# graphdeco-inria/reduced-3dgs

Hardware: AMD Instinct MI355X
Metric: train iters/s (fwd+bwd) + Mpix/s render, 500k Gaussians @1600x1062 (higher is better)
Workload: dtype f32

## Files before the change

reduced-3dgs_amd/csrc/common.h:

```cpp
#pragma once
#include <hip/hip_runtime.h>
#include <stddef.h>
#include <stdint.h>

#include <functional>
#include <stdexcept>
#include <string>

#include "gauss_math.h"
#include "param_math.h"

namespace r3 {

constexpr size_t kAlign = 256;
constexpr int kPairGrad = 9;
#ifndef R3_ACC_STRIDE
#define R3_ACC_STRIDE 12
#endif
#ifndef R3_PAIR_STRIDE
#define R3_PAIR_STRIDE 12
#endif
#ifdef R3_WP_VEC
constexpr int kPieceStride = 12;
#else
constexpr int kPieceStride = 9;
#endif
constexpr int kAccStride = R3_ACC_STRIDE;
constexpr int kPairStride = R3_PAIR_STRIDE;

constexpr int kPreBlockSize = 256;
struct PrePartial {
    uint32_t visible;
    uint32_t num_rendered;
    uint32_t depth_max;
    uint32_t depth_inv_min;
    uint32_t binned;
    uint32_t rendered_ref;
    uint32_t pad[2];
};
static_assert(sizeof(PrePartial) == 32, "two 16-byte loads per partial");
struct GeomHeader {
    uint32_t visible, num_rendered, depth_max, depth_inv_min;
    uint32_t num_pairs;
    uint32_t reserve;
    uint32_t sort_overflow;
    uint32_t binned;
    uint32_t rendered_ref;
    uint32_t sh_cache;
    uint32_t ckpt;
    uint32_t ckpt_thr;
    uint32_t pad[52];
};
static_assert(sizeof(GeomHeader) == 256, "header = 256 B");
inline size_t pre_partials(size_t P) { return (P + kPreBlockSize - 1) / kPreBlockSize; }

struct PassInfo {
    uint32_t seq;
    uint32_t num_rendered;
    uint32_t visible;
    uint32_t reserve;
    uint32_t sort_overflow;
    uint32_t sort_seq;
    uint32_t pairs;
    uint32_t pad;
};
static_assert(sizeof(PassInfo) == 32, "PassInfo = 32 B");

constexpr int kMinDepthBuckets = 1024;
constexpr int kMaxDepthBuckets = 16384;
constexpr int kBucketCap = 4096;
#ifndef R3_HIST_BATCH
#define R3_HIST_BATCH 4096
#endif
constexpr int kHistBatch = R3_HIST_BATCH;
inline size_t depth_hist_per_block(size_t P)
{
    const size_t want = (P + 255) / 256;
    const size_t per = ((want + kHistBatch - 1) / kHistBatch) * kHistBatch;
    return per < (size_t)kHistBatch ? (size_t)kHistBatch : per;
}
int depth_bucket_load();
inline int depth_bucket_count(size_t P)
{
    int nb = kMinDepthBuckets;
    const size_t load = (size_t)depth_bucket_load() * (P > (1u << 22) ? 8 : P > (1u << 20) ? 4 : 1);
    while (nb < kMaxDepthBuckets && P / (size_t)nb > load) nb <<= 1;
    return nb;
}
struct DepthSortScratch {
    uint32_t depth_max, depth_inv_min;
    uint32_t big_count, pad_;
    unsigned long long total[kMaxDepthBuckets + 1];
    uint32_t start[kMaxDepthBuckets + 2];
    uint32_t tile_base[kMaxDepthBuckets + 2];
    uint32_t big_list[kMaxDepthBuckets];
};
inline size_t depth_hist_rows(size_t P) { const size_t per = depth_hist_per_block(P); return (P + per - 1) / per; }

struct Carver {
    char* p;
    explicit Carver(char* base)
        : p(reinterpret_cast<char*>((reinterpret_cast<uintptr_t>(base) + kAlign - 1) & ~(uintptr_t)(kAlign - 1)))
    {
    }
    template <class T>
    T* take(size_t count)
    {
        T* r = reinterpret_cast<T*>(p);
        size_t bytes = (count * sizeof(T) + kAlign - 1) & ~(kAlign - 1);
        p += bytes;
        return r;
    }
};

struct GeomState {
    GeomHeader* header;
    PrePartial* partials;
    DepthSortScratch* dsort;
    unsigned long long* hist_rows;
    uint32_t* hist_base;
    GRec* rec;
    float* acc;
    ushort4* rect;
    uint32_t* depth_key;
    uint32_t* tiles;
    uint32_t* key_sorted;
    uint32_t* bucket_id;
    uint4* rec16;
    ushort4* rect_sorted;
    uint4* rec16_b;
    uint32_t* order;
    uint32_t* offsets;
    int* radii_internal;
    float* sh_ddir;
    uint32_t* ovf_key;
    uint32_t* ovf_id;
    char* temp;
    size_t temp_bytes;
    static GeomState carve(char* base, size_t P, size_t temp_bytes)
    {
        Carver c(base);
        GeomState g;
        const size_t nb = (size_t)depth_bucket_count(P);
        g.header = c.take<GeomHeader>(1);
        g.partials = c.take<PrePartial>(pre_partials(P));
        g.dsort = c.take<DepthSortScratch>(1);
        g.hist_rows = c.take<unsigned long long>(depth_hist_rows(P) * (nb + 1));
        g.hist_base = c.take<uint32_t>(depth_hist_rows(P) * (nb + 1));
        g.rec = c.take<GRec>(P);
        g.acc = c.take<float>(P * kAccStride);
        g.rect = c.take<ushort4>(P);
        g.depth_key = c.take<uint32_t>(P);
        g.tiles = c.take<uint32_t>(P);
        g.key_sorted = c.take<uint32_t>(P);
        g.bucket_id = c.take<uint32_t>(P);
        g.order = c.take<uint32_t>(P);
        g.offsets = c.take<uint32_t>(P);
        g.radii_internal = c.take<int>(P);
        g.ovf_key = c.take<uint32_t>(P);
        g.ovf_id = c.take<uint32_t>(P);
        g.rec16 = c.take<uint4>(P);
        g.rect_sorted = c.take<ushort4>(P);
        g.rec16_b = c.take<uint4>(P);
        g.temp = c.take<char>(temp_bytes);
        g.temp_bytes = temp_bytes;
        g.lean_end = c.p;
        g.sh_ddir = c.take<float>(P * 9);
        g.end = c.p;
        return g;
    }
    char* lean_end;
    char* end;
};

inline uint32_t higher_msb(uint32_t n)
{
    uint32_t msb = sizeof(n) * 4, step = msb;
    while (step > 1) {
        step /= 2;
        if (n >> msb)
            msb += step;
        else
            msb -= step;
    }
    if (n >> msb) msb++;
    return msb;
}

constexpr int kRadixBlock = 2048;
constexpr int kMaxRadixBins = 256;
constexpr int kMaxRadixPasses = 3;
struct PairLayout {
    int tile_bits;
    int rank_bits;
    int wide;
    int passes;
    int digit_bits;
};
PairLayout pair_layout(int P, size_t n_tiles);

inline uint32_t radix_row_stride(size_t R)
{
    return (uint32_t)(((R + kRadixBlock - 1) / kRadixBlock + 3) & ~(size_t)3);
}

constexpr int kBwdSegMinLog2 = 7;
constexpr int kBwdSegMaxLog2 = 8;
constexpr int kBwdSegMax = 32;
constexpr int kFwdCkptMax = 256;
constexpr uint32_t kUnitTileBits = 20;
R3_HD size_t ckpt_slot(uint32_t first, uint32_t k, uint32_t tile, uint32_t seg_log2) { return (size_t)(first >> seg_log2) + tile + k; }
inline size_t ckpt_slots(size_t R, size_t Tn) { return (R >> kBwdSegMinLog2) + Tn + 2; }
constexpr uint32_t kOrderLists = 8, kListBlock = 4, kListBlockTiles = kListBlock * kListBlock;
struct TileGrid {
    uint32_t gx, gy;
    R3_HD size_t n() const { return (size_t)gx * gy; }
    R3_HD uint32_t blocks_x() const { return (gx + kListBlock - 1) / kListBlock; }
    R3_HD uint32_t blocks() const { return blocks_x() * ((gy + kListBlock - 1) / kListBlock); }
    R3_HD uint32_t list_slots(uint32_t list) const
    {
        return blocks() > list ? (blocks() - list + kOrderLists - 1) / kOrderLists * kListBlockTiles : 0u;
    }
    R3_HD uint32_t list_tile(uint32_t list, uint32_t j) const
    {
        const uint32_t k = j / kListBlockTiles * kOrderLists + list, o = j % kListBlockTiles, bx = blocks_x();
        const uint32_t tx = k % bx * kListBlock + o % kListBlock, ty = k / bx * kListBlock + o / kListBlock;
        return tx < gx && ty < gy ? ty * gx + tx : 0xFFFFFFFFu;
    }
    R3_HD uint32_t list_tiles_max() const
    {
        const size_t m = (size_t)((blocks() + kOrderLists - 1) / kOrderLists) * kListBlockTiles;
        return (uint32_t)(m < n() ? m : n());
    }
};
R3_HD uint32_t bwd_list_fit(uint32_t pairs, const TileGrid& g)
{
    const size_t extra = (size_t)pairs >> kBwdSegMinLog2, most = 8 * g.n();
    return g.list_tiles_max() + (uint32_t)((extra < most ? extra : most) / kOrderLists);
}
inline uint32_t bwd_units_cap(uint32_t reserve, const TileGrid& g) { return (bwd_list_fit(reserve, g) + 1u) * kOrderLists; }
int bwd_segment_log2();
int bwd_segment_factor_pct();

struct BinState {
    uint32_t* point_list;
    float* pair_grad;
    float* wave_part;
    unsigned char* pair_flag;
    uint32_t* pair_rank;
    char* words_a;
    char* words_b;
    char* words_c;
    uint32_t* radix_rows;
    uint32_t* radix_base;
    uint32_t* radix_total;
    uint32_t* block_first;
    unsigned long long* quad_masks;
    uint32_t* unit_order;
    float4* ckpt;
    char* end;
    static BinState carve(char* base, size_t R, int wide, const TileGrid& grid)
    {
        const size_t Tn = grid.n();
        Carver c(base);
        BinState b;
        b.point_list = c.take<uint32_t>(R);
        b.pair_grad = c.take<float>(R * kPairStride);
        b.wave_part = c.take<float>((R / 64 + 1) * 2 * kPieceStride);
        b.pair_flag = c.take<unsigned char>(R);
        if (wide == 1) {
            b.pair_rank = c.take<uint32_t>(R);
            b.words_a = reinterpret_cast<char*>(c.take<unsigned long long>(R));
            b.words_b = reinterpret_cast<char*>(c.take<unsigned long long>(R));
            b.words_c = nullptr;
        } else if (wide == 2) {
            b.words_a = reinterpret_cast<char*>(c.take<unsigned long long>(R));
            b.words_b = reinterpret_cast<char*>(c.take<unsigned long long>(R));
            b.words_c = nullptr;
            b.pair_rank = reinterpret_cast<uint32_t*>(b.words_a);
        } else {
            b.words_a = reinterpret_cast<char*>(c.take<uint32_t>(R));
            b.words_b = reinterpret_cast<char*>(c.take<uint32_t>(R));
            b.words_c = reinterpret_cast<char*>(c.take<uint32_t>(R));
            b.pair_rank = reinterpret_cast<uint32_t*>(b.words_a);
        }
        b.radix_rows = c.take<uint32_t>((size_t)kMaxRadixBins * radix_row_stride(R));
        b.radix_base = c.take<uint32_t>((size_t)kMaxRadixBins * radix_row_stride(R));
        b.radix_total = c.take<uint32_t>(kMaxRadixPasses * kMaxRadixBins);
        b.quad_masks = c.take<unsigned long long>((R / 64 + Tn + 2) * 4);
        b.block_first = c.take<uint32_t>(R / kRadixBlock + 2);
        b.unit_order = c.take<uint32_t>((size_t)bwd_units_cap((uint32_t)R, grid) + 2 * kOrderLists);
        b.ckpt = c.take<float4>(ckpt_slots(R, Tn) * 256);
        b.end = c.p;
        return b;
    }
};

R3_HD size_t quad_mask_slot(uint32_t first, uint32_t chunk, uint32_t tile)
{
    return (size_t)(first >> 6) + chunk + tile;
}

struct ImageState {
    float* final_T;
    uint32_t* n_contrib;
    uint2* ranges;
    uint32_t* quad_depth;
    uint32_t* tile_order;
    char* end;
    static ImageState carve(char* base, size_t N, size_t Tn)
    {
        Carver c(base);
        ImageState s;
        s.final_T = c.take<float>(N);
        s.n_contrib = c.take<uint32_t>(N);
        s.ranges = c.take<uint2>(Tn);
        s.quad_depth = c.take<uint32_t>(Tn * 4);
        s.tile_order = c.take<uint32_t>(Tn);
        s.end = c.p;
        return s;
    }
};

template <class S, class... A>
size_t required_bytes(A... a)
{
    S s = S::carve(nullptr, a...);
    return (size_t)reinterpret_cast<uintptr_t>(s.end) + kAlign;
}

size_t depth_sort_temp_bytes(size_t P);

inline uint32_t grid_pairs_for(uint32_t reserve)
{
    const uint64_t g = (uint64_t)reserve * 7 / 10;
    return (uint32_t)(g < 1024 ? (reserve < 1024 ? reserve : 1024) : g);
}

struct Error : std::runtime_error {
    using std::runtime_error::runtime_error;
};

#if defined(__HIP_DEVICE_COMPILE__)
#define R3_GLOBAL __attribute__((address_space(1)))
#else
#define R3_GLOBAL
#endif
template <class T>
__device__ __forceinline__ R3_GLOBAL T* global_ptr(T* p)
{
    return (R3_GLOBAL T*)p;
}

int guarded_call(const std::function<int()>& f);

#define R3_HIP(expr)                                                                                   \
    do {                                                                                               \
        hipError_t e_ = (expr);                                                                        \
        if (e_ != hipSuccess)                                                                          \
            throw r3::Error(std::string(#expr) + " failed: " + hipGetErrorString(e_) + " (" + __FILE__ + \
                            ":" + std::to_string(__LINE__) + ")");                                     \
    } while (0)

inline void check_launch(const char* what, hipStream_t s, bool debug)
{
    hipError_t e = hipGetLastError();
    if (e != hipSuccess) throw Error(std::string(what) + ": launch failed: " + hipGetErrorString(e));
    if (debug) {
        e = hipStreamSynchronize(s);
        if (e != hipSuccess) throw Error(std::string(what) + ": " + hipGetErrorString(e));
    }
}

struct ViewParams {
    const float* view;
    const float* proj;
    const float* campos;
    const float* bg;
    float tan_fovx, tan_fovy;
    int W, H;
    float scale_modifier;
};

__device__ __forceinline__ Camera load_camera(const ViewParams& v)
{
    Camera c;
#pragma unroll
    for (int k = 0; k < 16; k++) {
        c.view[k] = v.view[k];
        c.proj[k] = v.proj[k];
    }
    c.campos[0] = v.campos[0];
    c.campos[1] = v.campos[1];
    c.campos[2] = v.campos[2];
    c.tan_fovx = v.tan_fovx;
    c.tan_fovy = v.tan_fovy;
    c.focal_y = v.H / (2.0f * v.tan_fovy);
    c.focal_x = v.W / (2.0f * v.tan_fovx);
    c.W = v.W;
    c.H = v.H;
    c.gx = (v.W + kTile - 1) / kTile;
    c.gy = (v.H + kTile - 1) / kTile;
    c.scale_modifier = v.scale_modifier;
    return c;
}

struct FwdInputs {
    int P, M;
    const int* degrees;
    const float* means3D;
    const float* scales;
    const float* rotations;
    const float* opacities;
    const float* shs;
    const float* cov3D_precomp;
    const float* colors_precomp;
    const int* coeffs_num;
    const int* per_band_count;
    const int* cumsum_count;
};

struct BwdOutputs {
    float* dL_dmean2D;
    float* dL_dopacity;
    float* dL_dcolor;
    float* dL_dmean3D;
    float* dL_dcov3D;
    float* dL_dsh;
    float* dL_dscale;
    float* dL_drot;
    float* dL_dconic;
};

struct PreArgs {
    FwdInputs in;
    ViewParams view;
    GRec* rec;
    ushort4* rect;
    uint32_t* depth_key;
    uint32_t* tiles;
    PrePartial* partials;
    int* radii;
    int color_blocks;
    int tight;
    float* sh_ddir;
};
struct HeaderArgs {
    const PrePartial* parts;
    int n_parts;
    GeomHeader* hdr;
    PassInfo* info;
    uint32_t ticket;
    uint32_t reserve;
    uint32_t stamp_sort;
    uint32_t sh_cache;
    uint32_t ckpt;
    uint32_t ckpt_factor_pct, n_tiles;
};
struct DepthArgs {
    int P, nb, rows, per_block;
    int fuse_header;
    const uint32_t* key;
    const uint32_t* tiles;
    GeomHeader* hdr;
    PassInfo* info;
    uint32_t ticket;
    DepthSortScratch* ds;
    unsigned long long* hist_rows;
    uint32_t* hist_base;
    uint32_t* key_sorted;
    uint32_t* bucket_id;
    uint32_t* ovf_key;
    uint32_t* ovf_id;
    const ushort4* rect;
    uint4* rec16;
    uint4* rec16_b;
    ushort4* rect_sorted;
    uint32_t* order;
    uint32_t* offsets;
    uint32_t* block_first;
    uint32_t block_cap;
};
struct EmitArgs {
    int P, gx;
    const GeomHeader* hdr;
    const uint32_t* order;
    const uint32_t* offsets;
    const uint32_t* block_first;
    const ushort4* rect;
    const ushort4* rect_sorted;
    GRec* rec;
    int rank_bits, digit_bits;
    char* words_out;
    uint32_t cap;
    uint32_t* pair_rank;
    uint2* ranges;
    uint32_t n_tiles;
    uint32_t* radix_rows;
    uint32_t row_stride;
};
struct RadixArgs {
    const GeomHeader* hdr;
    const char* in;
    char* out;
    uint32_t* ids_out;
    uint32_t cap;
    int shift, digit_bits;
    int rank_bits, tile_shift;
    uint32_t* rows;
    uint32_t* base;
    uint32_t* total;
    uint32_t row_stride;
};
struct RangesArgs {
    const GeomHeader* hdr;
    const char* sorted;
    uint32_t cap;
    int rank_bits;
    const uint32_t* order;
    uint32_t* point_list;
    uint2* ranges;
    unsigned char* pair_flag;
};
struct BlendFwdArgs {
    const uint2* ranges;
    const uint32_t* point_list;
    const GRec* rec;
    int W, H, gx;
    uint32_t nblocks;
    const float* bg;
    float* out_color;
    float* final_T;
    uint32_t* n_contrib;
    int* touched;
    float* transmittance;
    unsigned long long* quad_masks;
    uint32_t* quad_depth;
    float4* ckpt;
    const GeomHeader* hdr;
};
struct BlendBwdArgs {
    const uint2* ranges;
    const uint32_t* point_list;
    const GRec* rec;
    const float* final_T;
    const uint32_t* n_contrib;
    const float* dL_dpix;
    int W, H, gx;
    uint32_t nblocks;
    const float* bg;
    float* pair_grad;
    unsigned char* pair_flag;
    const unsigned long long* quad_masks;
    uint32_t* tile_order;
    uint32_t units_cap;
    const uint32_t* quad_depth;
    const float4* ckpt;
    const GeomHeader* hdr;
    int segments;
};
struct PairReduceArgs {
    const GeomHeader* hdr;
    const float* pair_grad;
    unsigned char* pair_flag;
    const uint32_t* pair_rank;
    uint32_t rank_mask;
    const uint32_t* order;
    const GRec* rec;
    const uint32_t* tiles;
    float* acc;
    float* wave_part;
    uint32_t stamp0, stamp1;
};
struct PreBwdArgs {
    FwdInputs in;
    ViewParams view;
    const int* radii;
    const GRec* rec;
    const uint32_t* tiles;
    const float* acc;
    const float* wave_part;
    const float* pair_grad;
    uint32_t stamp0, stamp1;
    const GeomHeader* header;
    float lambda_sh;
    const float* sh_ddir;
    int stagger;
    BwdOutputs out;
    const float* shs_rest;
    float* dL_dsh_rest;
};

struct FwdPassArgs {
    PreArgs pre;
    HeaderArgs header;
    DepthArgs depth;
    EmitArgs emit;
    RadixArgs radix[kMaxRadixPasses];
    RangesArgs ranges;
    BlendFwdArgs blend;
    const float* shs_rest;
};
struct BwdPassArgs {
    BlendBwdArgs blend;
    PairReduceArgs reduce;
    PreBwdArgs pre;
};
static_assert(sizeof(FwdPassArgs) <= 3072 && sizeof(BwdPassArgs) <= 3072, "pass blocks travel as by-value kernel arguments");

struct FwdPlan {
    int P, M, W, H, gx, gy;
    uint32_t reserve;
    uint32_t grid_pairs;
    PairLayout layout;
    int nb;
    int ragged, counters;
    int color_in_geom;
    int color_side;
    int fwd_ppl;
    int color_grid;
    int color_fuse;
    int color_split[3];
    int generic_depth_sort;
    int tight;
    int raw_params;
};
struct BwdPlan {
    int P, M, W, H, gx, gy;
    uint32_t reserve, grid_pairs;
    uint32_t units_cap;
    PairLayout layout;
    int bwd_ppl;
    int has_pairs;
    int f64_chain;
    int raw_params;
};

enum Stage { kPre = 0, kDepthSort, kBinning, kBlendFwd, kBlendBwd, kPreBwd, kColor, kBlendBwdKernel, kNumStages };

void issue_preprocess_geom(const FwdPlan& p, FwdPassArgs* dst, const FwdPassArgs& v, hipStream_t s);
void issue_preprocess_color(const FwdPlan& p, const PreArgs* a, hipStream_t s);
void launch_mark_visible(int P, const float* means3D, const float* view, bool* present, hipStream_t s);
void launch_activate_params(int P, const float* scaling_raw, const float* rotation_raw, float* scales, float* rotations,
                            hipStream_t s);

void issue_header_reduce(const HeaderArgs* a, hipStream_t s);
void prepare_depth_bucket_sort(int nb);
void issue_depth_sort_and_color(const FwdPlan& p, const FwdPassArgs* a, hipStream_t s);
void run_generic_depth_sort(int P, GeomState& g, hipStream_t s);
void issue_tile_binning(const FwdPlan& p, const FwdPassArgs* a, hipStream_t s);
const char* sorted_words(const BinState& b, const PairLayout& l);
void launch_export_keys(int P, int R, int cap, size_t n_tiles, const BinState& b, const GeomState& g, uint64_t* keys_out,
                        hipStream_t s);
void launch_export_point_list(int count, const uint32_t* point_list, const GeomHeader* hdr, uint32_t* out, hipStream_t s);

void issue_blend_forward(const FwdPlan& p, const BlendFwdArgs* a, hipStream_t s);
void issue_unit_order(const BwdPlan& p, BwdPassArgs* dst, const BwdPassArgs& v, hipStream_t s);
void issue_blend_backward(const BwdPlan& p, BwdPassArgs* dst, const BwdPassArgs& v, hipStream_t s);
void issue_pair_reduce(const BwdPlan& p, const PairReduceArgs* a, hipStream_t s);
void issue_preprocess_backward(const BwdPlan& p, const PreBwdArgs* a, hipStream_t s);

void launch_colour_variance_accumulate(int P, const int* D, int M, int max_sh_deg, const float* means3D,
                                       const float* cam_pos, const float* shs, const int* radii, const int* touched,
                                       const float* transmittance, float* wSum, float* wSumSq, float* mean,
                                       float* variance, float* accum, hipStream_t s);

int env_int(const char* env, int dflt, int lo, int hi);

#if defined(__HIPCC__)
template <class Block>
__device__ __forceinline__ void install_block_from_kernarg(Block* dst, int tid, int nthreads)
{
    static_assert(alignof(Block) == 8 && sizeof(Block) % 4 == 0, "kernarg layout: [dst (8 B)][block]");
#if defined(__HIP_DEVICE_COMPILE__)
    typedef const uint32_t __attribute__((address_space(4))) * KernargWords;
    KernargWords src = (KernargWords)__builtin_amdgcn_kernarg_segment_ptr() + sizeof(Block*) / 4;
    uint32_t* d = reinterpret_cast<uint32_t*>(dst);
    for (uint32_t k = (uint32_t)tid; k < sizeof(Block) / 4; k += (uint32_t)nthreads) d[k] = src[k];
#endif
}
#endif

}
```

reduced-3dgs_amd/csrc/preprocess_bwd.hip:

```cpp
#include "common.h"

namespace r3 {

#ifndef R3_PREBWD_BLOCK
#define R3_PREBWD_BLOCK 64
#endif
constexpr int kBwdBlock = R3_PREBWD_BLOCK;
constexpr int kBwdWaveShFloats = 64 * 48 + (64 * 48) / 32;

template <bool ROWS48>
__device__ __forceinline__ int bskew(int e)
{
    if (ROWS48) return e + (int)(((uint32_t)e * 43691u) >> 21);
    return e + (e >> 5);
}

template <bool ROWS48>
struct ShRowLdsRW {
    float* base;
    int roff;
    __device__ __forceinline__ float at(int e) const { return ROWS48 ? base[e] : base[bskew<false>(roff + e)]; }
    __device__ __forceinline__ void put(int e, float v) const
    {
        if (ROWS48)
            base[e] = v;
        else
            base[bskew<false>(roff + e)] = v;
    }
};

template <bool ROWS48>
__device__ __forceinline__ int split_lds_index(int f, int rl, int k0, int M)
{
    if (ROWS48) {
        const int row = k0 == 0 ? (int)(((uint32_t)f * 43691u) >> 17) : (int)(((uint32_t)f * 46604u) >> 21);
        return f + (49 - rl) * row + k0;
    }
    const int row = f / rl;
    return bskew<false>(row * 3 * M + k0 + (f - row * rl));
}

template <bool ROWS48, bool VEC>
__device__ __forceinline__ void stage_split_span(const float* __restrict__ src, int len, int rl, int k0, int M, float* lds,
                                                 int lane)
{
    if (VEC) {
        constexpr int kBatch = 6;
        const float4* src4 = reinterpret_cast<const float4*>(src);
        const int n4 = len >> 2;
        for (int base = 0; base < n4; base += 64 * kBatch) {
            float4 v[kBatch];
#pragma unroll
            for (int k = 0; k < kBatch; k++) {
                const int e4 = base + k * 64 + lane;
                v[k] = e4 < n4 ? src4[e4] : make_float4(0.f, 0.f, 0.f, 0.f);
            }
#pragma unroll
            for (int k = 0; k < kBatch; k++) {
                const int e4 = base + k * 64 + lane;
                if (e4 < n4) {
                    const int f = e4 << 2;
                    lds[split_lds_index<ROWS48>(f, rl, k0, M)] = v[k].x;
                    lds[split_lds_index<ROWS48>(f + 1, rl, k0, M)] = v[k].y;
                    lds[split_lds_index<ROWS48>(f + 2, rl, k0, M)] = v[k].z;
                    lds[split_lds_index<ROWS48>(f + 3, rl, k0, M)] = v[k].w;
                }
            }
        }
    } else {
        for (int f = lane; f < len; f += 64) lds[split_lds_index<ROWS48>(f, rl, k0, M)] = src[f];
    }
}

template <bool ROWS48, bool VEC>
__device__ __forceinline__ void unstage_split_span(float* __restrict__ dst, int len, int rl, int k0, int M, const float* lds,
                                                   int lane, bool rows)
{
    if (VEC) {
        float4* dst4 = reinterpret_cast<float4*>(dst);
        const int n4 = len >> 2;
        if (rows) {
            for (int e4 = lane; e4 < n4; e4 += 64) {
                const int f = e4 << 2;
                dst4[e4] = make_float4(lds[split_lds_index<ROWS48>(f, rl, k0, M)], lds[split_lds_index<ROWS48>(f + 1, rl, k0, M)],
                                       lds[split_lds_index<ROWS48>(f + 2, rl, k0, M)], lds[split_lds_index<ROWS48>(f + 3, rl, k0, M)]);
            }
        } else {
            for (int e4 = lane; e4 < n4; e4 += 64) dst4[e4] = make_float4(0.f, 0.f, 0.f, 0.f);
        }
    } else if (rows) {
        for (int f = lane; f < len; f += 64) dst[f] = lds[split_lds_index<ROWS48>(f, rl, k0, M)];
    } else {
        for (int f = lane; f < len; f += 64) dst[f] = 0.f;
    }
}

constexpr int kReduceGroups = 1;

__device__ __forceinline__ void pair_reduce_group(const PairReduceArgs& a, uint32_t e, int lane, bool valid, uint32_t key,
                                                  float (&v)[kPairGrad], uint32_t key_before, uint32_t key_after)
{
#define R3_SEG_STEP(CTRL, RMASK)                                                                                          \
    {                                                                                                                     \
        const uint32_t ku = (uint32_t)__builtin_amdgcn_update_dpp((int)~key, (int)key, CTRL, RMASK, 0xf, false);          \
        const bool take = ku == key;                                                                                      \
        _Pragma("unroll") for (int k = 0; k < kPairGrad; k++)                                                             \
        {                                                                                                                 \
            const float vu = __builtin_bit_cast(                                                                          \
                float, __builtin_amdgcn_update_dpp(0, __builtin_bit_cast(int, v[k]), CTRL, RMASK, 0xf, false));           \
            if (take) v[k] += vu;                                                                                         \
        }                                                                                                                 \
    }
    R3_SEG_STEP(0x111, 0xf)
    R3_SEG_STEP(0x112, 0xf)
    R3_SEG_STEP(0x114, 0xf)
    R3_SEG_STEP(0x118, 0xf)
    R3_SEG_STEP(0x142, 0xa)
    R3_SEG_STEP(0x143, 0xc)
#undef R3_SEG_STEP
    const uint32_t knext = (uint32_t)__shfl_down((int)key, 1);
    const uint32_t key0 = (uint32_t)__builtin_amdgcn_readfirstlane((int)key);
    if (valid && (lane == 63 || knext != key)) {
        const uint32_t gid = a.order ? a.order[key] : key;
        const bool from_before = key == key0 && key_before == key;
        const bool into_next = lane == 63 && key_after == key;
#ifdef R3_EXP_PR_NOSTORE
        if (v[0] != 12345.678f) return;
#endif
        if (!from_before && !into_next) {
#ifdef R3_ACC_IN_SLAB
            float4* dst = reinterpret_cast<float4*>(const_cast<float*>(a.pair_grad) + (size_t)e * kPairStride);
#else
            float4* dst = reinterpret_cast<float4*>(a.acc + (size_t)gid * kAccStride);
#endif
#ifndef R3_NO_ZERO_ROW_SKIP
            bool nz = false;
#pragma unroll
            for (int k = 0; k < kPairGrad; k++) nz |= v[k] != 0.f;
            if (nz) {
                dst[0] = make_float4(v[0], v[1], v[2], v[3]);
                dst[1] = make_float4(v[4], v[5], v[6], v[7]);
                dst[2] = make_float4(v[8], __uint_as_float(a.stamp0), __uint_as_float(a.stamp1), 0.f);
            }
#else
            dst[0] = make_float4(v[0], v[1], v[2], v[3]);
            dst[1] = make_float4(v[4], v[5], v[6], v[7]);
            dst[2] = make_float4(v[8], 0.f, 0.f, 0.f);
            if (kAccStride >= 16) dst[3] = make_float4(0.f, 0.f, 0.f, 0.f);
#endif
        } else {
            float* wp = a.wave_part + (size_t)(e >> 6) * 2 * kPieceStride;
#ifdef R3_WP_VEC
            if (from_before) {
                float4* w4 = reinterpret_cast<float4*>(wp);
                w4[0] = make_float4(v[0], v[1], v[2], v[3]);
                w4[1] = make_float4(v[4], v[5], v[6], v[7]);
                w4[2] = make_float4(v[8], 0.f, 0.f, 0.f);
            }
            if (into_next) {
                float4* w4 = reinterpret_cast<float4*>(wp + kPieceStride);
                w4[0] = make_float4(v[0], v[1], v[2], v[3]);
                w4[1] = make_float4(v[4], v[5], v[6], v[7]);
                w4[2] = make_float4(v[8], 0.f, 0.f, 0.f);
            }
#else
            if (from_before) {
#pragma unroll
                for (int k = 0; k < kPairGrad; k++) wp[k] = v[k];
            }
            if (into_next) {
#pragma unroll
                for (int k = 0; k < kPairGrad; k++) wp[kPieceStride + k] = v[k];
            }
#endif
        }
    }
}

#ifdef R3_PR_WAVES
__attribute__((amdgpu_waves_per_eu(R3_PR_WAVES, R3_PR_WAVES)))
#endif
__global__ __launch_bounds__(256) void pair_reduce_kernel(const PairReduceArgs* __restrict__ ap)
{
    const PairReduceArgs a = *ap;
    const uint32_t R = a.hdr->num_pairs;
    constexpr uint32_t kPerBlock = 256u * kReduceGroups;
  for (uint32_t blk = blockIdx.x; blk * kPerBlock < R; blk += gridDim.x) {
    const float* __restrict__ pair_grad = a.pair_grad;
    unsigned char* __restrict__ pair_flag = a.pair_flag;
    const uint32_t* __restrict__ pair_gid = a.pair_rank;
    const uint32_t rank_mask = a.rank_mask;
    const int lane = threadIdx.x & 63, wave = threadIdx.x >> 6;
    const uint32_t e0 = blk * kPerBlock + (uint32_t)wave * (64u * kReduceGroups) + (uint32_t)lane;
    float v[kReduceGroups][kPairGrad];
    uint32_t key[kReduceGroups], kb[kReduceGroups], ka[kReduceGroups];
    bool flag[kReduceGroups];
#pragma unroll
    for (int g = 0; g < kReduceGroups; g++) {
        const uint32_t e = e0 + 64u * g, gbase = e & ~63u;
        key[g] = e < R ? pair_gid[e] & rank_mask : 0xFFFFFFFFu;
        flag[g] = e < R && pair_flag[e] != 0;
        kb[g] = gbase > 0u && gbase < R ? pair_gid[gbase - 1u] & rank_mask : 0xFFFFFFFFu;
        ka[g] = gbase + 64u < R ? pair_gid[gbase + 64u] & rank_mask : 0xFFFFFFFFu;
    }
#pragma unroll
    for (int g = 0; g < kReduceGroups; g++) {
        const uint32_t e = e0 + 64u * g;
#pragma unroll
        for (int k = 0; k < kPairGrad; k++) v[g][k] = 0.f;
#ifdef R3_EXP_PR_NOLOAD
        if (flag[g] && e == 0xFFFFFFF0u) {
#else
        if (flag[g]) {
#endif
            pair_flag[e] = 0;
            const float4* src = reinterpret_cast<const float4*>(pair_grad + (size_t)e * kPairStride);
            const float4 r0 = src[0], r1 = src[1];
            v[g][0] = r0.x; v[g][1] = r0.y; v[g][2] = r0.z; v[g][3] = r0.w;
            v[g][4] = r1.x; v[g][5] = r1.y; v[g][6] = r1.z; v[g][7] = r1.w;
            v[g][8] = src[2].x;
        }
    }
#pragma unroll
    for (int g = 0; g < kReduceGroups; g++) {
        const uint32_t e = e0 + 64u * g;
        pair_reduce_group(a, e, lane, e < R, key[g], v[g], kb[g], ka[g]);
    }
  }
}

void issue_pair_reduce(const BwdPlan& p, const PairReduceArgs* a, hipStream_t s)
{
    if (!p.has_pairs) return;
    constexpr uint32_t per = 256u * kReduceGroups;
    hipLaunchKernelGGL(pair_reduce_kernel, dim3((p.grid_pairs + per - 1u) / per), dim3(256), 0, s, a);
}

template <bool ROWS48, bool F64, bool RAW = false>
__global__ __launch_bounds__(kBwdBlock) void preprocess_bwd_kernel(const PreBwdArgs* __restrict__ ap)
{
    __shared__ float s_sh[kBwdBlock / 64][kBwdWaveShFloats];
    const PreBwdArgs a = *ap;
    const int tid = threadIdx.x, lane = tid & 63, wave = tid >> 6;
    const int P = a.in.P, M = a.in.M;
    const int i = blockIdx.x * kBwdBlock + tid;
    const bool valid = i < P;
    const int wave_first = blockIdx.x * kBwdBlock + wave * 64;
    const Camera cam = load_camera(a.view);
    const bool has_sh = a.in.shs != nullptr;

    const bool vis = valid && a.radii[i] > 0;
    const int nrows = max(0, min(64, P - wave_first));
    const int span_len = has_sh ? nrows * 3 * M : 0;
    const long span_first = 3L * M * wave_first;
    float* lds = s_sh[wave];
    const bool wave_vis = __ballot(vis) != 0ull;
    const bool cached = has_sh && a.sh_ddir != nullptr && a.header->sh_cache != 0u;
    if (!cached && a.stagger > 0 && blockIdx.x < 768u * (256 / kBwdBlock)) {
        const int steps = (int)(blockIdx.x / (256u * (256 / kBwdBlock))) * a.stagger;
        for (int k = 0; k < steps; k += 127) __builtin_amdgcn_s_sleep(127);
    }
    if (RAW) {
        if (wave_vis && !cached) {
            const int rl = 3 * (M - 1);
            if ((nrows & 3) == 0) {
                stage_split_span<ROWS48, true>(a.in.shs + 3L * wave_first, 3 * nrows, 3, 0, M, lds, lane);
                if (M > 1) stage_split_span<ROWS48, true>(a.shs_rest + (long)rl * wave_first, rl * nrows, rl, 3, M, lds, lane);
            } else {
                stage_split_span<ROWS48, false>(a.in.shs + 3L * wave_first, 3 * nrows, 3, 0, M, lds, lane);
                if (M > 1) stage_split_span<ROWS48, false>(a.shs_rest + (long)rl * wave_first, rl * nrows, rl, 3, M, lds, lane);
            }
        }
    } else if (has_sh && wave_vis && !cached) {
        const float* src = a.in.shs + span_first;
        if (((span_first | span_len) & 3) == 0) {
            const float4* src4 = reinterpret_cast<const float4*>(src);
            const int n4 = span_len >> 2;
            constexpr int kBatch = 6;
            for (int base = 0; base < n4; base += 64 * kBatch) {
                float4 v[kBatch];
#pragma unroll
                for (int k = 0; k < kBatch; k++) {
                    const int e4 = base + k * 64 + lane;
                    v[k] = e4 < n4 ? src4[e4] : make_float4(0.f, 0.f, 0.f, 0.f);
                }
#pragma unroll
                for (int k = 0; k < kBatch; k++) {
                    const int e4 = base + k * 64 + lane;
                    if (e4 < n4) {
                        const int e = e4 << 2;
                        if (ROWS48) {
                            float* d = lds + bskew<true>(e);
                            d[0] = v[k].x;
                            d[1] = v[k].y;
                            d[2] = v[k].z;
                            d[3] = v[k].w;
                        } else {
                            lds[bskew<false>(e)] = v[k].x;
                            lds[bskew<false>(e + 1)] = v[k].y;
                            lds[bskew<false>(e + 2)] = v[k].z;
                            lds[bskew<false>(e + 3)] = v[k].w;
                        }
                    }
                }
            }
        } else {
            for (int e = lane; e < span_len; e += 64) lds[bskew<ROWS48>(e)] = src[e];
        }
    }
    __syncthreads();

    float dmean[3] = {0.f, 0.f, 0.f}, dcov6[6] = {0.f, 0.f, 0.f, 0.f, 0.f, 0.f};
    float dscale[3] = {0.f, 0.f, 0.f}, dq[4] = {0.f, 0.f, 0.f, 0.f};
    float g2x = 0.f, g2y = 0.f, dop = 0.f, dcol[3] = {0.f, 0.f, 0.f}, gcon[3] = {0.f, 0.f, 0.f};
    int K = 0;
    const ShRowLdsRW<ROWS48> row{ROWS48 ? lds + 49 * lane : lds, ROWS48 ? 0 : lane * 3 * M};
    if (vis) {
        const float mx = a.in.means3D[3 * i], my = a.in.means3D[3 * i + 1], mz = a.in.means3D[3 * i + 2];
        const GRec r = a.rec[i];
        const uint32_t start = r.pair_start, ntile = a.tiles[i];
        if (a.wave_part && start != 0xFFFFFFFFu && start + ntile <= a.header->num_pairs) {
            float acc9[kPairGrad];
            const uint32_t last = start + ntile - 1u;
            const uint32_t w0 = start >> 6, w1 = last >> 6;
            if (w0 == w1) {
#ifdef R3_ACC_IN_SLAB
                const float4* ap = reinterpret_cast<const float4*>(a.pair_grad + (size_t)last * kPairStride);
#else
                const float4* ap = reinterpret_cast<const float4*>(a.acc + (size_t)i * kAccStride);
#endif
                float4 a0 = ap[0], a1 = ap[1], a2 = ap[2];
#ifndef R3_NO_ZERO_ROW_SKIP
                if (__float_as_uint(a2.y) != a.stamp0 || __float_as_uint(a2.z) != a.stamp1)
                    a0 = a1 = a2 = make_float4(0.f, 0.f, 0.f, 0.f);
#endif
                acc9[0] = a0.x; acc9[1] = a0.y; acc9[2] = a0.z; acc9[3] = a0.w;
                acc9[4] = a1.x; acc9[5] = a1.y; acc9[6] = a1.z; acc9[7] = a1.w;
                acc9[8] = a2.x;
            } else {
#ifdef R3_WP_VEC
                const float4* w4 = reinterpret_cast<const float4*>(a.wave_part + (size_t)w0 * 2 * kPieceStride + kPieceStride);
                float4 p0 = w4[0], p1 = w4[1], p2 = w4[2];
                acc9[0] = p0.x; acc9[1] = p0.y; acc9[2] = p0.z; acc9[3] = p0.w;
                acc9[4] = p1.x; acc9[5] = p1.y; acc9[6] = p1.z; acc9[7] = p1.w;
                acc9[8] = p2.x;
                for (uint32_t w = w0 + 1; w <= w1; w++) {
                    w4 = reinterpret_cast<const float4*>(a.wave_part + (size_t)w * 2 * kPieceStride);
                    p0 = w4[0]; p1 = w4[1]; p2 = w4[2];
                    acc9[0] += p0.x; acc9[1] += p0.y; acc9[2] += p0.z; acc9[3] += p0.w;
                    acc9[4] += p1.x; acc9[5] += p1.y; acc9[6] += p1.z; acc9[7] += p1.w;
                    acc9[8] += p2.x;
                }
#else
                const float* wp = a.wave_part + (size_t)w0 * 2 * kPieceStride + kPieceStride;
#pragma unroll
                for (int k = 0; k < kPairGrad; k++) acc9[k] = wp[k];
                for (uint32_t w = w0 + 1; w <= w1; w++) {
                    wp = a.wave_part + (size_t)w * 2 * kPieceStride;
#pragma unroll
                    for (int k = 0; k < kPairGrad; k++) acc9[k] += wp[k];
                }
#endif
            }
            g2x = acc9[0];
            g2y = acc9[1];
            gcon[0] = acc9[2];
            gcon[1] = acc9[3];
            gcon[2] = acc9[4];
            dop = acc9[5];
            dcol[0] = acc9[6];
            dcol[1] = acc9[7];
            dcol[2] = acc9[8];
        }
        float sc[3] = {0.f, 0.f, 0.f}, q[4] = {1.f, 0.f, 0.f, 0.f}, c6[6];
        float qn = 1.f;
        if (a.in.cov3D_precomp) {
            for (int k = 0; k < 6; k++) c6[k] = a.in.cov3D_precomp[6 * i + k];
        } else {
            for (int k = 0; k < 3; k++) sc[k] = a.in.scales[3 * i + k];
            for (int k = 0; k < 4; k++) q[k] = a.in.rotations[4 * i + k];
            if (RAW) {
                const float rq[4] = {q[0], q[1], q[2], q[3]};
                for (int k = 0; k < 3; k++) sc[k] = scale_act(sc[k]);
                qn = quat_act(rq, q);
            }
            cov3d_from_scale_rot(sc, cam.scale_modifier, q, c6);
        }
        double dcov6d[6];
        if (F64) {
            cov2d_backward_f64(cam, mx, my, mz, c6, gcon[0], gcon[1], gcon[2], dcov6d, dmean);
#pragma unroll
            for (int k = 0; k < 6; k++) dcov6[k] = (float)dcov6d[k];
        } else {
            cov2d_backward(cam, mx, my, mz, c6, gcon[0], gcon[1], gcon[2], dcov6, dmean);
        }
        project_backward(cam, mx, my, mz, g2x, g2y, dmean);
        if (has_sh) {
            float mult = 0.f;
            if (a.lambda_sh != 0.f) {
                const uint32_t V = a.header->visible;
                mult = a.lambda_sh / (float)((int)V * 15 * 3);
            }
            const int deg = a.in.degrees[i];
            K = (deg + 1) * (deg + 1);
            if (cached) {
                float d9[9];
#pragma unroll
                for (int k = 0; k < 9; k++)
                    d9[k] = (deg > 0 && ntile > 0u) ? a.sh_ddir[9 * (size_t)i + k] : 0.f;
                sh_backward<true>(deg, row, row, d9, mx, my, mz, cam.campos, r.width_clamp >> 16, dcol, 0.f, dmean);
            } else {
                sh_backward<false>(deg, row, row, nullptr, mx, my, mz, cam.campos, r.width_clamp >> 16, dcol, mult, dmean);
            }
        }
        if (a.in.scales) {
            if (F64)
                cov3d_backward_f64(sc, cam.scale_modifier, q, dcov6d, dscale, dq);
            else
                cov3d_backward(sc, cam.scale_modifier, q, dcov6, dscale, dq);
            if (RAW) {
                for (int k = 0; k < 3; k++) dscale[k] = scale_act_bwd(dscale[k], sc[k]);
                const float gq[4] = {dq[0], dq[1], dq[2], dq[3]};
                quat_act_bwd(q, qn, gq, dq);
            }
        }
        dop = opacity_backward(dop, r.op);
    }
    if (has_sh && valid) {
        if (wave_vis) {
            for (int e = 3 * K; e < 3 * M; e++) row.put(e, 0.f);
        }
    }
    __syncthreads();
    if (RAW) {
        const int rl = 3 * (M - 1);
        if ((nrows & 3) == 0) {
            unstage_split_span<ROWS48, true>(a.out.dL_dsh + 3L * wave_first, 3 * nrows, 3, 0, M, lds, lane, wave_vis);
            if (M > 1)
                unstage_split_span<ROWS48, true>(a.dL_dsh_rest + (long)rl * wave_first, rl * nrows, rl, 3, M, lds, lane, wave_vis);
        } else {
            unstage_split_span<ROWS48, false>(a.out.dL_dsh + 3L * wave_first, 3 * nrows, 3, 0, M, lds, lane, wave_vis);
            if (M > 1)
                unstage_split_span<ROWS48, false>(a.dL_dsh_rest + (long)rl * wave_first, rl * nrows, rl, 3, M, lds, lane, wave_vis);
        }
    } else if (has_sh) {
        float* dst = a.out.dL_dsh + span_first;
        if (((span_first | span_len) & 3) == 0) {
            float4* dst4 = reinterpret_cast<float4*>(dst);
            const int n4 = span_len >> 2;
            if (wave_vis) {
                for (int e4 = lane; e4 < n4; e4 += 64) {
                    const int e = e4 << 2;
                    if (ROWS48) {
                        const float* q = lds + bskew<true>(e);
                        dst4[e4] = make_float4(q[0], q[1], q[2], q[3]);
                    } else {
                        dst4[e4] = make_float4(lds[bskew<false>(e)], lds[bskew<false>(e + 1)], lds[bskew<false>(e + 2)],
                                               lds[bskew<false>(e + 3)]);
                    }
                }
            } else {
                for (int e4 = lane; e4 < n4; e4 += 64) dst4[e4] = make_float4(0.f, 0.f, 0.f, 0.f);
            }
        } else if (wave_vis) {
            for (int e = lane; e < span_len; e += 64) dst[e] = lds[bskew<ROWS48>(e)];
        } else {
            for (int e = lane; e < span_len; e += 64) dst[e] = 0.f;
        }
    }
    if (valid) {
        float* o;
        o = a.out.dL_dmean2D + 3 * (size_t)i;
        o[0] = g2x;
        o[1] = g2y;
        o[2] = 0.f;
        a.out.dL_dopacity[i] = dop;
        o = a.out.dL_dcolor + 3 * (size_t)i;
        o[0] = dcol[0];
        o[1] = dcol[1];
        o[2] = dcol[2];
        o = a.out.dL_dmean3D + 3 * (size_t)i;
        o[0] = dmean[0];
        o[1] = dmean[1];
        o[2] = dmean[2];
        o = a.out.dL_dcov3D + 6 * (size_t)i;
        for (int k = 0; k < 6; k++) o[k] = dcov6[k];
        o = a.out.dL_dscale + 3 * (size_t)i;
        o[0] = dscale[0];
        o[1] = dscale[1];
        o[2] = dscale[2];
        o = a.out.dL_drot + 4 * (size_t)i;
        o[0] = dq[0];
        o[1] = dq[1];
        o[2] = dq[2];
        o[3] = dq[3];
        if (a.out.dL_dconic) {
            o = a.out.dL_dconic + 4 * (size_t)i;
            o[0] = gcon[0];
            o[1] = gcon[1];
            o[2] = 0.f;
            o[3] = gcon[2];
        }
    }
}

void issue_preprocess_backward(const BwdPlan& p, const PreBwdArgs* a, hipStream_t s)
{
    const int blocks = (p.P + kBwdBlock - 1) / kBwdBlock;
    static const int lds_pad = env_int("R3DGS_PREBWD_LDS_PAD", 0, 0, 65536);
    if (p.raw_params) {
        if (p.M == 16) {
            if (p.f64_chain)
                hipLaunchKernelGGL((preprocess_bwd_kernel<true, true, true>), dim3(blocks), dim3(kBwdBlock), lds_pad, s, a);
            else
                hipLaunchKernelGGL((preprocess_bwd_kernel<true, false, true>), dim3(blocks), dim3(kBwdBlock), lds_pad, s, a);
        } else {
            if (p.f64_chain)
                hipLaunchKernelGGL((preprocess_bwd_kernel<false, true, true>), dim3(blocks), dim3(kBwdBlock), lds_pad, s, a);
            else
                hipLaunchKernelGGL((preprocess_bwd_kernel<false, false, true>), dim3(blocks), dim3(kBwdBlock), lds_pad, s, a);
        }
        return;
    }
    if (p.M == 16) {
        if (p.f64_chain)
            hipLaunchKernelGGL((preprocess_bwd_kernel<true, true>), dim3(blocks), dim3(kBwdBlock), lds_pad, s, a);
        else
            hipLaunchKernelGGL((preprocess_bwd_kernel<true, false>), dim3(blocks), dim3(kBwdBlock), lds_pad, s, a);
    } else {
        if (p.f64_chain)
            hipLaunchKernelGGL((preprocess_bwd_kernel<false, true>), dim3(blocks), dim3(kBwdBlock), lds_pad, s, a);
        else
            hipLaunchKernelGGL((preprocess_bwd_kernel<false, false>), dim3(blocks), dim3(kBwdBlock), lds_pad, s, a);
    }
}

}
```

Measured before the change: 1560.

## Hoist per-lane loads to kernel entry and tag pointers as global address space

Pointers in the preprocess-backward and pair-reduce kernels are now marked with a global address-space qualifier, so the compiler can emit global memory instructions instead of flat ones. All per-Gaussian inputs (record, tile count, accumulator row, means, scales, rotations, degree, cached SH direction terms, header fields) are loaded at kernel start, before the SH staging and its barrier. The aim is to overlap these loads' latency with the LDS staging. The cost is higher register pressure from the live values, which may reduce occupancy.

```diff
diff --git a/reduced-3dgs_amd/csrc/common.h b/reduced-3dgs_amd/csrc/common.h
--- a/reduced-3dgs_amd/csrc/common.h
+++ b/reduced-3dgs_amd/csrc/common.h
@@ -382,17 +382,18 @@
     float scale_modifier;
 };
 
-__device__ __forceinline__ Camera load_camera(const ViewParams& v)
+template <class Ptr>
+__device__ __forceinline__ Camera load_camera_from(Ptr view, Ptr proj, Ptr campos, const ViewParams& v)
 {
     Camera c;
 #pragma unroll
     for (int k = 0; k < 16; k++) {
-        c.view[k] = v.view[k];
-        c.proj[k] = v.proj[k];
-    }
-    c.campos[0] = v.campos[0];
-    c.campos[1] = v.campos[1];
-    c.campos[2] = v.campos[2];
+        c.view[k] = view[k];
+        c.proj[k] = proj[k];
+    }
+    c.campos[0] = campos[0];
+    c.campos[1] = campos[1];
+    c.campos[2] = campos[2];
     c.tan_fovx = v.tan_fovx;
     c.tan_fovy = v.tan_fovy;
     c.focal_y = v.H / (2.0f * v.tan_fovy);
@@ -404,6 +405,7 @@
     c.scale_modifier = v.scale_modifier;
     return c;
 }
+__device__ __forceinline__ Camera load_camera(const ViewParams& v) { return load_camera_from(v.view, v.proj, v.campos, v); }
 
 struct FwdInputs {
     int P, M;
diff --git a/reduced-3dgs_amd/csrc/preprocess_bwd.hip b/reduced-3dgs_amd/csrc/preprocess_bwd.hip
--- a/reduced-3dgs_amd/csrc/preprocess_bwd.hip
+++ b/reduced-3dgs_amd/csrc/preprocess_bwd.hip
@@ -41,19 +41,20 @@
 }
 
 template <bool ROWS48, bool VEC>
-__device__ __forceinline__ void stage_split_span(const float* __restrict__ src, int len, int rl, int k0, int M, float* lds,
+__device__ __forceinline__ void stage_split_span(const R3_GLOBAL float* __restrict__ src, int len, int rl, int k0, int M, float* lds,
                                                  int lane)
 {
     if (VEC) {
         constexpr int kBatch = 6;
-        const float4* src4 = reinterpret_cast<const float4*>(src);
+        const R3_GLOBAL float4* src4 = reinterpret_cast<const R3_GLOBAL float4*>(src);
         const int n4 = len >> 2;
         for (int base = 0; base < n4; base += 64 * kBatch) {
             float4 v[kBatch];
 #pragma unroll
             for (int k = 0; k < kBatch; k++) {
                 const int e4 = base + k * 64 + lane;
-                v[k] = e4 < n4 ? src4[e4] : make_float4(0.f, 0.f, 0.f, 0.f);
+                v[k] = make_float4(0.f, 0.f, 0.f, 0.f);
+                if (e4 < n4) v[k] = src4[e4];
             }
 #pragma unroll
             for (int k = 0; k < kBatch; k++) {
@@ -73,11 +74,11 @@
 }
 
 template <bool ROWS48, bool VEC>
-__device__ __forceinline__ void unstage_split_span(float* __restrict__ dst, int len, int rl, int k0, int M, const float* lds,
+__device__ __forceinline__ void unstage_split_span(R3_GLOBAL float* __restrict__ dst, int len, int rl, int k0, int M, const float* lds,
                                                    int lane, bool rows)
 {
     if (VEC) {
-        float4* dst4 = reinterpret_cast<float4*>(dst);
+        R3_GLOBAL float4* dst4 = reinterpret_cast<R3_GLOBAL float4*>(dst);
         const int n4 = len >> 2;
         if (rows) {
             for (int e4 = lane; e4 < n4; e4 += 64) {
@@ -121,7 +122,7 @@
     const uint32_t knext = (uint32_t)__shfl_down((int)key, 1);
     const uint32_t key0 = (uint32_t)__builtin_amdgcn_readfirstlane((int)key);
     if (valid && (lane == 63 || knext != key)) {
-        const uint32_t gid = a.order ? a.order[key] : key;
+        const uint32_t gid = a.order ? global_ptr(a.order)[key] : key;
         const bool from_before = key == key0 && key_before == key;
         const bool into_next = lane == 63 && key_after == key;
 #ifdef R3_EXP_PR_NOSTORE
@@ -129,9 +130,9 @@
 #endif
         if (!from_before && !into_next) {
 #ifdef R3_ACC_IN_SLAB
-            float4* dst = reinterpret_cast<float4*>(const_cast<float*>(a.pair_grad) + (size_t)e * kPairStride);
+            auto* dst = reinterpret_cast<R3_GLOBAL float4*>(global_ptr(const_cast<float*>(a.pair_grad)) + (size_t)e * kPairStride);
 #else
-            float4* dst = reinterpret_cast<float4*>(a.acc + (size_t)gid * kAccStride);
+            auto* dst = reinterpret_cast<R3_GLOBAL float4*>(global_ptr(a.acc) + (size_t)gid * kAccStride);
 #endif
 #ifndef R3_NO_ZERO_ROW_SKIP
             bool nz = false;
@@ -149,16 +150,16 @@
             if (kAccStride >= 16) dst[3] = make_float4(0.f, 0.f, 0.f, 0.f);
 #endif
         } else {
-            float* wp = a.wave_part + (size_t)(e >> 6) * 2 * kPieceStride;
+            R3_GLOBAL float* wp = global_ptr(a.wave_part) + (size_t)(e >> 6) * 2 * kPieceStride;
 #ifdef R3_WP_VEC
             if (from_before) {
-                float4* w4 = reinterpret_cast<float4*>(wp);
+                auto* w4 = reinterpret_cast<R3_GLOBAL float4*>(wp);
                 w4[0] = make_float4(v[0], v[1], v[2], v[3]);
                 w4[1] = make_float4(v[4], v[5], v[6], v[7]);
                 w4[2] = make_float4(v[8], 0.f, 0.f, 0.f);
             }
             if (into_next) {
-                float4* w4 = reinterpret_cast<float4*>(wp + kPieceStride);
+                auto* w4 = reinterpret_cast<R3_GLOBAL float4*>(wp + kPieceStride);
                 w4[0] = make_float4(v[0], v[1], v[2], v[3]);
                 w4[1] = make_float4(v[4], v[5], v[6], v[7]);
                 w4[2] = make_float4(v[8], 0.f, 0.f, 0.f);
@@ -183,12 +184,12 @@
 __global__ __launch_bounds__(256) void pair_reduce_kernel(const PairReduceArgs* __restrict__ ap)
 {
     const PairReduceArgs a = *ap;
-    const uint32_t R = a.hdr->num_pairs;
+    const uint32_t R = global_ptr(a.hdr)->num_pairs;
     constexpr uint32_t kPerBlock = 256u * kReduceGroups;
   for (uint32_t blk = blockIdx.x; blk * kPerBlock < R; blk += gridDim.x) {
-    const float* __restrict__ pair_grad = a.pair_grad;
-    unsigned char* __restrict__ pair_flag = a.pair_flag;
-    const uint32_t* __restrict__ pair_gid = a.pair_rank;
+    const R3_GLOBAL float* __restrict__ pair_grad = global_ptr(a.pair_grad);
+    R3_GLOBAL unsigned char* __restrict__ pair_flag = global_ptr(a.pair_flag);
+    const R3_GLOBAL uint32_t* __restrict__ pair_gid = global_ptr(a.pair_rank);
     const uint32_t rank_mask = a.rank_mask;
     const int lane = threadIdx.x & 63, wave = threadIdx.x >> 6;
     const uint32_t e0 = blk * kPerBlock + (uint32_t)wave * (64u * kReduceGroups) + (uint32_t)lane;
@@ -214,7 +215,7 @@
         if (flag[g]) {
 #endif
             pair_flag[e] = 0;
-            const float4* src = reinterpret_cast<const float4*>(pair_grad + (size_t)e * kPairStride);
+            const auto* src = reinterpret_cast<const R3_GLOBAL float4*>(pair_grad + (size_t)e * kPairStride);
             const float4 r0 = src[0], r1 = src[1];
             v[g][0] = r0.x; v[g][1] = r0.y; v[g][2] = r0.z; v[g][3] = r0.w;
             v[g][4] = r1.x; v[g][5] = r1.y; v[g][6] = r1.z; v[g][7] = r1.w;
@@ -246,16 +247,63 @@
     const int i = blockIdx.x * kBwdBlock + tid;
     const bool valid = i < P;
     const int wave_first = blockIdx.x * kBwdBlock + wave * 64;
-    const Camera cam = load_camera(a.view);
+    const Camera cam = load_camera_from(global_ptr(a.view.view), global_ptr(a.view.proj), global_ptr(a.view.campos), a.view);
     const bool has_sh = a.in.shs != nullptr;
-
-    const bool vis = valid && a.radii[i] > 0;
+    const auto* hdr = global_ptr(a.header);
+    const uint32_t num_pairs = hdr->num_pairs, n_visible = hdr->visible, hdr_sh_cache = hdr->sh_cache;
+    const bool cached = has_sh && a.sh_ddir != nullptr && hdr_sh_cache != 0u;
+
+#ifndef R3_PREBWD_LOAD_CULLED
+#define R3_PREBWD_LOAD_CULLED 0
+#endif
+    int radius = 0, deg = 0;
+    uint32_t ntile = 0u;
+    GRec r;
+    float4 a0, a1, a2;
+    float m3[3], sc[3], q[4], c6[6], d9in[9];
+    const auto load_lane = [&]() {
+        r = global_ptr(a.rec)[i];
+        ntile = global_ptr(a.tiles)[i];
+#ifndef R3_ACC_IN_SLAB
+        const auto* arow = reinterpret_cast<const R3_GLOBAL float4*>(global_ptr(a.acc) + (size_t)i * kAccStride);
+        a0 = arow[0];
+        a1 = arow[1];
+        a2 = arow[2];
+#endif
+        for (int k = 0; k < 3; k++) m3[k] = global_ptr(a.in.means3D)[3 * i + k];
+        if (!a.in.cov3D_precomp) {
+            for (int k = 0; k < 3; k++) sc[k] = global_ptr(a.in.scales)[3 * i + k];
+            for (int k = 0; k < 4; k++) q[k] = global_ptr(a.in.rotations)[4 * i + k];
+        }
+        if (has_sh) deg = global_ptr(a.in.degrees)[i];
+        if (cached) {
+#pragma unroll
+            for (int k = 0; k < 9; k++) d9in[k] = global_ptr(a.sh_ddir)[9 * (size_t)i + k];
+        }
+        if (a.in.cov3D_precomp) {
+            for (int k = 0; k < 6; k++) c6[k] = global_ptr(a.in.cov3D_precomp)[6 * i + k];
+            sc[0] = sc[1] = sc[2] = 0.f;
+            q[0] = 1.f;
+            q[1] = q[2] = q[3] = 0.f;
+        }
+    };
+#if R3_PREBWD_LOAD_CULLED
+    if (valid) {
+        radius = global_ptr(a.radii)[i];
+        load_lane();
+    }
+    const bool vis = valid && radius > 0;
+#else
+    if (valid) radius = global_ptr(a.radii)[i];
+    const bool vis = valid && radius > 0;
+    if (vis) load_lane();
+#endif
+
     const int nrows = max(0, min(64, P - wave_first));
     const int span_len = has_sh ? nrows * 3 * M : 0;
     const long span_first = 3L * M * wave_first;
     float* lds = s_sh[wave];
     const bool wave_vis = __ballot(vis) != 0ull;
-    const bool cached = has_sh && a.sh_ddir != nullptr && a.header->sh_cache != 0u;
     if (!cached && a.stagger > 0 && blockIdx.x < 768u * (256 / kBwdBlock)) {
         const int steps = (int)(blockIdx.x / (256u * (256 / kBwdBlock))) * a.stagger;
         for (int k = 0; k < steps; k += 127) __builtin_amdgcn_s_sleep(127);
@@ -263,18 +311,20 @@
     if (RAW) {
         if (wave_vis && !cached) {
             const int rl = 3 * (M - 1);
+            const auto* dc = global_ptr(a.in.shs) + 3L * wave_first;
+            const auto* rest = global_ptr(a.shs_rest) + (long)rl * wave_first;
             if ((nrows & 3) == 0) {
-                stage_split_span<ROWS48, true>(a.in.shs + 3L * wave_first, 3 * nrows, 3, 0, M, lds, lane);
-                if (M > 1) stage_split_span<ROWS48, true>(a.shs_rest + (long)rl * wave_first, rl * nrows, rl, 3, M, lds, lane);
+                stage_split_span<ROWS48, true>(dc, 3 * nrows, 3, 0, M, lds, lane);
+                if (M > 1) stage_split_span<ROWS48, true>(rest, rl * nrows, rl, 3, M, lds, lane);
             } else {
-                stage_split_span<ROWS48, false>(a.in.shs + 3L * wave_first, 3 * nrows, 3, 0, M, lds, lane);
-                if (M > 1) stage_split_span<ROWS48, false>(a.shs_rest + (long)rl * wave_first, rl * nrows, rl, 3, M, lds, lane);
+                stage_split_span<ROWS48, false>(dc, 3 * nrows, 3, 0, M, lds, lane);
+                if (M > 1) stage_split_span<ROWS48, false>(rest, rl * nrows, rl, 3, M, lds, lane);
             }
         }
     } else if (has_sh && wave_vis && !cached) {
-        const float* src = a.in.shs + span_first;
+        const R3_GLOBAL float* src = global_ptr(a.in.shs) + span_first;
         if (((span_first | span_len) & 3) == 0) {
-            const float4* src4 = reinterpret_cast<const float4*>(src);
+            const auto* src4 = reinterpret_cast<const R3_GLOBAL float4*>(src);
             const int n4 = span_len >> 2;
             constexpr int kBatch = 6;
             for (int base = 0; base < n4; base += 64 * kBatch) {
@@ -282,7 +332,8 @@
 #pragma unroll
                 for (int k = 0; k < kBatch; k++) {
                     const int e4 = base + k * 64 + lane;
-                    v[k] = e4 < n4 ? src4[e4] : make_float4(0.f, 0.f, 0.f, 0.f);
+                    v[k] = make_float4(0.f, 0.f, 0.f, 0.f);
+                    if (e4 < n4) v[k] = src4[e4];
                 }
 #pragma unroll
                 for (int k = 0; k < kBatch; k++) {
@@ -316,20 +367,19 @@
     int K = 0;
     const ShRowLdsRW<ROWS48> row{ROWS48 ? lds + 49 * lane : lds, ROWS48 ? 0 : lane * 3 * M};
     if (vis) {
-        const float mx = a.in.means3D[3 * i], my = a.in.means3D[3 * i + 1], mz = a.in.means3D[3 * i + 2];
-        const GRec r = a.rec[i];
-        const uint32_t start = r.pair_start, ntile = a.tiles[i];
-        if (a.wave_part && start != 0xFFFFFFFFu && start + ntile <= a.header->num_pairs) {
+        const float mx = m3[0], my = m3[1], mz = m3[2];
+        const uint32_t start = r.pair_start;
+        if (a.wave_part && start != 0xFFFFFFFFu && start + ntile <= num_pairs) {
             float acc9[kPairGrad];
             const uint32_t last = start + ntile - 1u;
             const uint32_t w0 = start >> 6, w1 = last >> 6;
             if (w0 == w1) {
 #ifdef R3_ACC_IN_SLAB
-                const float4* ap = reinterpret_cast<const float4*>(a.pair_grad + (size_t)last * kPairStride);
-#else
-                const float4* ap = reinterpret_cast<const float4*>(a.acc + (size_t)i * kAccStride);
-#endif
-                float4 a0 = ap[0], a1 = ap[1], a2 = ap[2];
+                const auto* arow = reinterpret_cast<const R3_GLOBAL float4*>(global_ptr(a.pair_grad) + (size_t)last * kPairStride);
+                a0 = arow[0];
+                a1 = arow[1];
+                a2 = arow[2];
+#endif
 #ifndef R3_NO_ZERO_ROW_SKIP
                 if (__float_as_uint(a2.y) != a.stamp0 || __float_as_uint(a2.z) != a.stamp1)
                     a0 = a1 = a2 = make_float4(0.f, 0.f, 0.f, 0.f);
@@ -338,25 +388,26 @@
                 acc9[4] = a1.x; acc9[5] = a1.y; acc9[6] = a1.z; acc9[7] = a1.w;
                 acc9[8] = a2.x;
             } else {
+                const R3_GLOBAL float* wave_part = global_ptr(a.wave_part);
 #ifdef R3_WP_VEC
-                const float4* w4 = reinterpret_cast<const float4*>(a.wave_part + (size_t)w0 * 2 * kPieceStride + kPieceStride);
+                const auto* w4 = reinterpret_cast<const R3_GLOBAL float4*>(wave_part + (size_t)w0 * 2 * kPieceStride + kPieceStride);
                 float4 p0 = w4[0], p1 = w4[1], p2 = w4[2];
                 acc9[0] = p0.x; acc9[1] = p0.y; acc9[2] = p0.z; acc9[3] = p0.w;
                 acc9[4] = p1.x; acc9[5] = p1.y; acc9[6] = p1.z; acc9[7] = p1.w;
                 acc9[8] = p2.x;
                 for (uint32_t w = w0 + 1; w <= w1; w++) {
-                    w4 = reinterpret_cast<const float4*>(a.wave_part + (size_t)w * 2 * kPieceStride);
+                    w4 = reinterpret_cast<const R3_GLOBAL float4*>(wave_part + (size_t)w * 2 * kPieceStride);
                     p0 = w4[0]; p1 = w4[1]; p2 = w4[2];
                     acc9[0] += p0.x; acc9[1] += p0.y; acc9[2] += p0.z; acc9[3] += p0.w;
                     acc9[4] += p1.x; acc9[5] += p1.y; acc9[6] += p1.z; acc9[7] += p1.w;
                     acc9[8] += p2.x;
                 }
 #else
-                const float* wp = a.wave_part + (size_t)w0 * 2 * kPieceStride + kPieceStride;
+                const R3_GLOBAL float* wp = wave_part + (size_t)w0 * 2 * kPieceStride + kPieceStride;
 #pragma unroll
                 for (int k = 0; k < kPairGrad; k++) acc9[k] = wp[k];
                 for (uint32_t w = w0 + 1; w <= w1; w++) {
-                    wp = a.wave_part + (size_t)w * 2 * kPieceStride;
+                    wp = wave_part + (size_t)w * 2 * kPieceStride;
 #pragma unroll
                     for (int k = 0; k < kPairGrad; k++) acc9[k] += wp[k];
                 }
@@ -372,13 +423,8 @@
             dcol[1] = acc9[7];
             dcol[2] = acc9[8];
         }
-        float sc[3] = {0.f, 0.f, 0.f}, q[4] = {1.f, 0.f, 0.f, 0.f}, c6[6];
         float qn = 1.f;
-        if (a.in.cov3D_precomp) {
-            for (int k = 0; k < 6; k++) c6[k] = a.in.cov3D_precomp[6 * i + k];
-        } else {
-            for (int k = 0; k < 3; k++) sc[k] = a.in.scales[3 * i + k];
-            for (int k = 0; k < 4; k++) q[k] = a.in.rotations[4 * i + k];
+        if (!a.in.cov3D_precomp) {
             if (RAW) {
                 const float rq[4] = {q[0], q[1], q[2], q[3]};
                 for (int k = 0; k < 3; k++) sc[k] = scale_act(sc[k]);
@@ -397,17 +443,13 @@
         project_backward(cam, mx, my, mz, g2x, g2y, dmean);
         if (has_sh) {
             float mult = 0.f;
-            if (a.lambda_sh != 0.f) {
-                const uint32_t V = a.header->visible;
-                mult = a.lambda_sh / (float)((int)V * 15 * 3);
-            }
-            const int deg = a.in.degrees[i];
+            if (a.lambda_sh != 0.f) mult = a.lambda_sh / (float)((int)n_visible * 15 * 3);
             K = (deg + 1) * (deg + 1);
             if (cached) {
                 float d9[9];
 #pragma unroll
                 for (int k = 0; k < 9; k++)
-                    d9[k] = (deg > 0 && ntile > 0u) ? a.sh_ddir[9 * (size_t)i + k] : 0.f;
+                    d9[k] = (deg > 0 && ntile > 0u) ? d9in[k] : 0.f;
                 sh_backward<true>(deg, row, row, d9, mx, my, mz, cam.campos, r.width_clamp >> 16, dcol, 0.f, dmean);
             } else {
                 sh_backward<false>(deg, row, row, nullptr, mx, my, mz, cam.campos, r.width_clamp >> 16, dcol, mult, dmean);
@@ -434,19 +476,19 @@
     __syncthreads();
     if (RAW) {
         const int rl = 3 * (M - 1);
+        R3_GLOBAL float* dc = global_ptr(a.out.dL_dsh) + 3L * wave_first;
+        R3_GLOBAL float* rest = global_ptr(a.dL_dsh_rest) + (long)rl * wave_first;
         if ((nrows & 3) == 0) {
-            unstage_split_span<ROWS48, true>(a.out.dL_dsh + 3L * wave_first, 3 * nrows, 3, 0, M, lds, lane, wave_vis);
-            if (M > 1)
-                unstage_split_span<ROWS48, true>(a.dL_dsh_rest + (long)rl * wave_first, rl * nrows, rl, 3, M, lds, lane, wave_vis);
-        } else {
-            unstage_split_span<ROWS48, false>(a.out.dL_dsh + 3L * wave_first, 3 * nrows, 3, 0, M, lds, lane, wave_vis);
-            if (M > 1)
-                unstage_split_span<ROWS48, false>(a.dL_dsh_rest + (long)rl * wave_first, rl * nrows, rl, 3, M, lds, lane, wave_vis);
+            unstage_split_span<ROWS48, true>(dc, 3 * nrows, 3, 0, M, lds, lane, wave_vis);
+            if (M > 1) unstage_split_span<ROWS48, true>(rest, rl * nrows, rl, 3, M, lds, lane, wave_vis);
+        } else {
+            unstage_split_span<ROWS48, false>(dc, 3 * nrows, 3, 0, M, lds, lane, wave_vis);
+            if (M > 1) unstage_split_span<ROWS48, false>(rest, rl * nrows, rl, 3, M, lds, lane, wave_vis);
         }
     } else if (has_sh) {
-        float* dst = a.out.dL_dsh + span_first;
+        R3_GLOBAL float* dst = global_ptr(a.out.dL_dsh) + span_first;
         if (((span_first | span_len) & 3) == 0) {
-            float4* dst4 = reinterpret_cast<float4*>(dst);
+            auto* dst4 = reinterpret_cast<R3_GLOBAL float4*>(dst);
             const int n4 = span_len >> 2;
             if (wave_vis) {
                 for (int e4 = lane; e4 < n4; e4 += 64) {
@@ -469,33 +511,33 @@
         }
     }
     if (valid) {
-        float* o;
-        o = a.out.dL_dmean2D + 3 * (size_t)i;
+        R3_GLOBAL float* o;
+        o = global_ptr(a.out.dL_dmean2D) + 3 * (size_t)i;
         o[0] = g2x;
         o[1] = g2y;
         o[2] = 0.f;
-        a.out.dL_dopacity[i] = dop;
-        o = a.out.dL_dcolor + 3 * (size_t)i;
+        global_ptr(a.out.dL_dopacity)[i] = dop;
+        o = global_ptr(a.out.dL_dcolor) + 3 * (size_t)i;
         o[0] = dcol[0];
         o[1] = dcol[1];
         o[2] = dcol[2];
-        o = a.out.dL_dmean3D + 3 * (size_t)i;
+        o = global_ptr(a.out.dL_dmean3D) + 3 * (size_t)i;
         o[0] = dmean[0];
         o[1] = dmean[1];
         o[2] = dmean[2];
-        o = a.out.dL_dcov3D + 6 * (size_t)i;
+        o = global_ptr(a.out.dL_dcov3D) + 6 * (size_t)i;
         for (int k = 0; k < 6; k++) o[k] = dcov6[k];
-        o = a.out.dL_dscale + 3 * (size_t)i;
+        o = global_ptr(a.out.dL_dscale) + 3 * (size_t)i;
         o[0] = dscale[0];
         o[1] = dscale[1];
         o[2] = dscale[2];
-        o = a.out.dL_drot + 4 * (size_t)i;
+        o = global_ptr(a.out.dL_drot) + 4 * (size_t)i;
         o[0] = dq[0];
         o[1] = dq[1];
         o[2] = dq[2];
         o[3] = dq[3];
         if (a.out.dL_dconic) {
-            o = a.out.dL_dconic + 4 * (size_t)i;
+            o = global_ptr(a.out.dL_dconic) + 4 * (size_t)i;
             o[0] = gcon[0];
             o[1] = gcon[1];
             o[2] = 0.f;
```

New measurement: 1585, median of 6. +1.6%, better.
